# EvolEcolGroup/tidypopgen

Hardware: AMD Instinct MI355X
Metric: SNP-genotypes/s (N x M) for IBS+KING+GRM+Fst+PCA; max |delta| vs CPU ref (cpu_baseline.parity) (higher is better)
Workload: dtype fp4-e2m1 operands (exact integers, f32 accumulate) for the cross-products, the PCA Gram and the grouped counts, int8 (int32 accumulate) for the loadings, f64 for statistics

## Files before the change

tidypopgen_amd/csrc/pca.hip:

```cpp
#include <math.h>
#include <stdio.h>
#include <stdlib.h>
#include <string.h>
#include <time.h>

#include <algorithm>

#include "common.h"
#include <type_traits>
#include "devfrag.h"

#define MFMA_I8(a, b, c) __builtin_amdgcn_mfma_i32_32x32x32_i8((a), (b), (c), 0, 0, 0)
#define PCA_NAN __longlong_as_double(0x7FF8000000000000ll)

__global__ void tpg_pca_center_scale_kernel(const int4* __restrict__ counts, int64_t m, int64_t n,
                                            double* __restrict__ center, double* __restrict__ scale,
                                            int* __restrict__ flags) {
  for (int64_t j = blockIdx.x * (int64_t)blockDim.x + threadIdx.x; j < m; j += (int64_t)gridDim.x * blockDim.x) {
    const int4 c = counts[j];
    if (c.w != 0) flags[0] = 1;
    const double mean = (double)(c.y + 2 * c.z) / (double)n;
    const double p = mean / 2;
    const double sd = sqrt(2 * p * (1 - p));
    if (!(sd > 0)) flags[1] = 1;
// ... 963 lines not shown
      for (int c = 0; c < 8; c++) {
        const int j = cg * 8 + c;
        const double x = j < p ? xs[i + j * p] : 0.0;
        a0[c] += a * x;
        a1[c] += y * x;
      }
    }
#pragma unroll
  for (int c = 0; c < 8; c++) {
    const int j = cg * 8 + c;
    double r = 0;
    if (live && j < p) {
      Y0[row + (int64_t)j * n] = a0[c];
      Y1[row + (int64_t)j * n] = a1[c];
      r = ldexp(a1[c] - theta[j] * a0[c], -e1);
      r *= r;
    }
#pragma unroll
    for (int off = 16; off >= 1; off >>= 1) r += __shfl_xor(r, off, 32);
    if ((threadIdx.x & 31) == 0 && j < p) rpart[(int64_t)blockIdx.x * p + j] = r;
  }
}

__global__ void tpg_fill_random_kernel(double* __restrict__ Q, int64_t total, uint64_t seed) {
  for (int64_t idx = blockIdx.x * (int64_t)blockDim.x + threadIdx.x; idx < total; idx += (int64_t)gridDim.x * blockDim.x) {
    uint64_t x = (uint64_t)idx * 0x9E3779B97F4A7C15ull + seed;
    x = (x ^ (x >> 30)) * 0xBF58476D1CE4E5B9ull;
    x = (x ^ (x >> 27)) * 0x94D049BB133111EBull;
    x ^= x >> 31;
    Q[idx] = (double)(int64_t)(x >> 11) * (1.0 / 9007199254740992.0) - 0.5;
  }
}

#include "host/host_eig.h"

struct EigWork {
  tpg_ctx* ctx;
  const double* K;
  int n, b, S;
  double *part = nullptr, *gpart = nullptr;
  int nchunks, rows_per_chunk;
  const double* L = nullptr;
  int nl = 0;
  double *lam_dev = nullptr, *cdev = nullptr, *dtmp = nullptr;
  double* xdev = nullptr;
  DevArena mem;
  TpgPcaOp* op = nullptr;
  int init() {
    const int row_blocks = (n + 63) / 64;
    S = 1;
    while (row_blocks * S < 4 * ctx->num_cu && S < 32 && n / (S * 2) >= 64) S *= 2;
    S = std::max(1, std::min((int)S, 2 * ctx->num_cu / row_blocks));
    if (op) S = 1;
    rows_per_chunk = n <= 4096 ? 32 : 64;
    nchunks = (n + rows_per_chunk - 1) / rows_per_chunk;
    TPG_TRY(mem.get(&part, (size_t)S * (size_t)b * (size_t)n));
    TPG_TRY(mem.get(&gpart, (size_t)nchunks * 64 * 64));
    TPG_TRY(mem.get(&lam_dev, 64));
    TPG_TRY(mem.get(&cdev, 64 * 64));
    TPG_TRY(mem.get(&dtmp, (size_t)b * (size_t)n));
    TPG_TRY(mem.get(&xdev, 64 * 64 + 64));
    return TPG_OK;
  }
  int set_locked(const double* Lptr, int count, const double* lam_host) {
    L = Lptr;
    nl = count;
    if (count > 0) TPG_HIP(tpg_push_small(ctx, lam_dev, lam_host, sizeof(double) * (size_t)count));
    return TPG_OK;
  }
  int apply(const double* Q, double alpha, const double* Y1, double beta, const double* Y0, double gamma, double* Y) {
    if (op) {
      TPG_TRY(tpg_pcaop_apply(ctx, op, Q, b, part));
    } else {
      dim3 grid((unsigned)((n + 63) / 64), (unsigned)S);
      TPG_LAUNCH(ctx, "eig_symm_apply", tpg_symm_apply_kernel, grid, dim3(256), 0, K, n, Q, b, S, part);
    }
    const double* Dm = nullptr;
    if (nl > 0) {
      TPG_LAUNCH(ctx, "eig_gram_small", tpg_gram_small_kernel, dim3((unsigned)nchunks), dim3(256), 0, L, nl, Q, b, n,
                 rows_per_chunk, gpart);
      TPG_LAUNCH(ctx, "eig_gram_reduce", tpg_gram_reduce_kernel, dim3((unsigned)((nl * b + 63) / 64)), dim3(256), 0,
                 (const double*)gpart, nchunks, nl, b, (const double*)lam_dev, cdev);
      TPG_LAUNCH(ctx, "eig_right_mult", tpg_right_mult_kernel, dim3((unsigned)((n + 31) / 32)), dim3(256), 0, L, n, nl,
                 (const double*)cdev, b, dtmp);
      Dm = dtmp;
    }
    TPG_LAUNCH(ctx, "eig_combine", tpg_combine_kernel, dim3(1024), dim3(256), 0, (const double*)part, S,
               (int64_t)n * b, alpha, Y1, beta, Y0, gamma, Y, Dm);
    TPG_CHECK_LAUNCH();
    return TPG_OK;
  }
  int gram(const double* A, int p, const double* B, int bb, std::vector<double>& C) {
    TPG_LAUNCH(ctx, "eig_gram_small", tpg_gram_small_kernel, dim3((unsigned)nchunks), dim3(256), 0, A, p, B, bb, n,
               rows_per_chunk, gpart);
    TPG_LAUNCH(ctx, "eig_gram_reduce", tpg_gram_reduce_kernel, dim3((unsigned)((p * bb + 63) / 64)), dim3(256), 0,
               (const double*)gpart, nchunks, p, bb, (const double*)nullptr, cdev);
    C.assign((size_t)p * bb, 0.0);
    TPG_HIP(tpg_fetch_small(ctx, C.data(), cdev, sizeof(double) * (size_t)p * bb));
    return TPG_OK;
  }
  int ritz(const double* A, const double* Yk, int p, const std::vector<double>& X, const std::vector<double>& theta, int e1,
           double* Y0, double* Y1, std::vector<double>& res2) {
    double* dx = xdev;
    TPG_HIP(tpg_push_small(ctx, dx, X.data(), sizeof(double) * (size_t)p * p));
    TPG_HIP(tpg_push_small(ctx, dx + 64 * 64, theta.data(), sizeof(double) * (size_t)p));
    const int nblk = (n + 31) / 32;
    TPG_LAUNCH(ctx, "eig_ritz", tpg_ritz_kernel, dim3((unsigned)nblk), dim3(256), 0, A, Yk, n, p, (const double*)dx,
               (const double*)(dx + 64 * 64), e1, Y0, Y1, gpart);
    TPG_LAUNCH(ctx, "eig_gram_reduce", tpg_gram_reduce_kernel, dim3((unsigned)((p + 63) / 64)), dim3(256), 0,
               (const double*)gpart, nblk, p, 1, (const double*)nullptr, cdev);
    res2.assign((size_t)p, 0.0);
    TPG_HIP(tpg_fetch_small(ctx, res2.data(), cdev, sizeof(double) * (size_t)p));
    return TPG_OK;
  }
  int rmult(const double* A, int p, const std::vector<double>& X, int b2, double* Y) {
    double* dx = xdev;
    TPG_HIP(tpg_push_small(ctx, dx, X.data(), sizeof(double) * (size_t)p * b2));
    TPG_LAUNCH(ctx, "eig_right_mult", tpg_right_mult_kernel, dim3((unsigned)((n + 31) / 32)), dim3(256), 0, A, n, p,
               (const double*)dx, b2, Y);
    TPG_CHECK_LAUNCH();
    return TPG_OK;
  }
};

struct StageTimer {
  tpg_ctx* ctx; const char* tag; bool on; double t0;
  static double now() { struct timespec ts; clock_gettime(CLOCK_MONOTONIC, &ts); return ts.tv_sec * 1e3 + ts.tv_nsec * 1e-6; }
  StageTimer(tpg_ctx* c, const char* t) : ctx(c), tag(t), on(tpg_env_set("TPG_DEBUG")), t0(0) { if (on) { (void)hipStreamSynchronize(ctx->stream); t0 = now(); } }
  void mark(const char* what) {
    if (!on) return;
    (void)hipStreamSynchronize(ctx->stream);
    const double t1 = now();
    fprintf(stderr, "[%s] %-28s %8.3f ms\n", tag, what, t1 - t0);
    t0 = t1;
  }
};

static int eig_topk(tpg_ctx* ctx, const double* d_K, int n, int k, double* lambda_host, double* d_U, double tol = 1e-12,
                    const double* d_P = nullptr, int np_ = 0, double* lam1_io = nullptr, TpgPcaOp* op = nullptr) {
  int b = 2 * k + 12;
  b = tpg_env_int("TPG_EIG_BLOCK", b);
  if (b > 64) b = 64;
  if (b > n - np_) b = n - np_;
  TPG_REQUIRE(k <= b, TPG_EINVAL, "k = %d too large (at most %d components)", k, b);
  TPG_REQUIRE(!op || b <= op->bmax, TPG_EINVAL, "block of %d columns, operator scratch for %d", b, op->bmax);
  EigWork w{ctx, d_K, n, b, 1};
  w.op = op;
  TPG_TRY(w.init());
  double *Q = nullptr, *Y = nullptr, *Y0 = nullptr, *Y1 = nullptr;
  for (double** blk : {&Q, &Y, &Y0, &Y1}) TPG_TRY(w.mem.get(blk, (size_t)n * (size_t)b));
  auto colbytes = [&](int cols) { return sizeof(double) * (size_t)n * (size_t)cols; };
  auto axpby = [&](const double* x, double alpha, const double* y, double beta, double* out, int cols) -> int {
    TPG_LAUNCH(ctx, "eig_combine", tpg_combine_kernel, dim3(1024), dim3(256), 0, x, 1, (int64_t)n * cols, alpha, y,
               beta, (const double*)nullptr, 0.0, out, (const double*)nullptr);
    TPG_CHECK_LAUNCH();
    return TPG_OK;
  };

  auto project_earlier = [&](double* A, int cols, double* tmp) -> int {
    for (int c0 = 0; c0 < np_; c0 += 64) {
      const int pc = std::min(64, np_ - c0);
      const double* P = d_P + (size_t)n * (size_t)c0;
      std::vector<double> Cm;
      TPG_TRY(w.gram(P, pc, A, cols, Cm));
      TPG_TRY(w.rmult(P, pc, Cm, cols, tmp));
      TPG_TRY(axpby(tmp, -1.0, A, 1.0, A, cols));
    }
    return TPG_OK;
  };

  auto orthonormalize = [&](double* A, int act, const double* L, int nl, double* tmp, int passes = 2) -> int {
    int extra_passes = 0;
    for (int pass = 0; pass < passes; pass++) {
      TPG_TRY(project_earlier(A, act, tmp));
      if (nl > 0) {
        std::vector<double> Cm;
        TPG_TRY(w.gram(L, nl, A, act, Cm));
        TPG_TRY(w.rmult(L, nl, Cm, act, tmp));
        TPG_TRY(axpby(tmp, -1.0, A, 1.0, A, act));
      }
      std::vector<double> G, Ri;
      TPG_TRY(w.gram(A, act, A, act, G));
      std::vector<double> D((size_t)act);
      for (int j = 0; j < act; j++) D[(size_t)j] = G[j + (size_t)j * act] > 0 ? 1.0 / sqrt(G[j + (size_t)j * act]) : 1.0;
      for (int j = 0; j < act; j++)
        for (int i = 0; i < act; i++) G[i + (size_t)j * act] *= D[(size_t)i] * D[(size_t)j];
      std::vector<double> Gsave = G;
      if (host_cholesky_upper(G, act)) {
        host_upper_inverse(G, act, Ri);
      } else {
        std::vector<double> lamg, Vg;
        host_sym_eig(Gsave, act, lamg, Vg);
        if (tpg_env_set("TPG_DEBUG")) fprintf(stderr, "[eig] CholQR fell back to the eigen-decomposition of the block Gram matrix\n");
        const double floor_ = std::max(lamg[0], 1e-300) * 1e-14;
        Ri.assign((size_t)act * act, 0.0);
        for (int j = 0; j < act; j++) {
          const double sc = 1.0 / sqrt(std::max(lamg[(size_t)j], floor_));
          for (int i = 0; i < act; i++) Ri[i + (size_t)j * act] = Vg[i + (size_t)j * act] * sc;
        }
        if (pass == passes - 1) pass = passes - 2, extra_passes++;
        if (extra_passes > 3) { tpg_set_error("eigen solver: block lost rank"); return TPG_ENUMERIC; }
      }
      for (int j = 0; j < act; j++)
        for (int i = 0; i < act; i++) Ri[i + (size_t)j * act] *= D[(size_t)i];
      TPG_TRY(w.rmult(A, act, Ri, act, tmp));
      TPG_HIP(tpg_copy_dev(ctx, A, tmp, colbytes(act)));
    }
    return TPG_OK;
  };

  StageTimer st(ctx, "eig");
  TPG_LAUNCH(ctx, "eig_random", tpg_fill_random_kernel, dim3(512), dim3(256), 0, Q, (int64_t)n * b, (uint64_t)0x5EED);
  TPG_TRY(orthonormalize(Q, b, nullptr, 0, Y, np_ > 0 ? 2 : 1));
  st.mark("init + orthonormalize");
  std::vector<double> lam((size_t)b, 0.0), theta, X, H;
  int nl = 0;
  const int MAXIT = 200;
  const double TOL = tol, AMP = 1e6;
  const bool own_scale = !(lam1_io && *lam1_io > 0);
  double lam1 = own_scale ? 0 : *lam1_io;
  int e1 = 0;
  for (int it = 0; it < MAXIT && nl < k; it++) {
    const int act = b - nl;
    double* A = Q + (size_t)n * nl;
    w.b = act;
    TPG_TRY(w.set_locked(Q, nl, lam.data()));
    TPG_TRY(w.apply(A, 1.0, nullptr, 0, nullptr, 0, Y));
    TPG_TRY(project_earlier(Y, act, Y0));
    TPG_TRY(w.gram(A, act, Y, act, H));
    st.mark("apply + gram(H)");
    for (int i = 0; i < act; i++)
      for (int j = i + 1; j < act; j++) {
        const double sy = 0.5 * (H[i + (size_t)j * act] + H[j + (size_t)i * act]);
        H[i + (size_t)j * act] = sy;
        H[j + (size_t)i * act] = sy;
      }
    const bool first = it == 0 && b < n - np_;
    host_sym_eig(H, act, theta, X, !first);
    st.mark("host_sym_eig");
    std::vector<double> RR;
    if (first) {
      if (own_scale) lam1 = fabs(theta[0]) > 0 ? fabs(theta[0]) : 1.0;
    } else {
      if (own_scale && nl == 0) lam1 = fabs(theta[0]) > 0 ? fabs(theta[0]) : 1.0;
      frexp(lam1, &e1);
      TPG_TRY(w.ritz(A, Y, act, X, theta, e1, Y0, Y1, RR));
      TPG_HIP(tpg_copy_dev(ctx, A, Y0, colbytes(act)));
      st.mark("ritz vectors + residuals");
    }
    const double lam1s = ldexp(lam1, -e1);
    int newly = 0;
    while (!first && newly < act && nl + newly < k && sqrt(std::max(0.0, RR[(size_t)newly])) < TOL * lam1s) newly++;
    for (int j = 0; j < newly; j++) lam[(size_t)(nl + j)] = theta[(size_t)j];
    nl += newly;
    if (nl >= k) break;
    const int act2 = b - nl;
    TPG_REQUIRE(act2 >= 2, TPG_ENUMERIC, "eigen solver ran out of active vectors");
    double* A2 = Q + (size_t)n * nl;
    const double* KA2 = first ? Y : Y1 + (size_t)n * newly;
    const double up = std::max(theta[(size_t)act - 1], 1e-300 * lam1), lo = 0.0;
    const double a0 = std::max(theta[(size_t)newly], up * (1 + 1e-8));
    const double ec = (up - lo) / 2, cc = (up + lo) / 2;
    const double x0 = (a0 - cc) / ec;
    int deg = 20;
    if (x0 > 1.0 + 1e-12) {
      const double dmax = log(2 * AMP) / acosh(x0);
      deg = dmax < 2 ? 2 : (dmax > 20 ? 20 : (int)dmax);
    }
    if (tpg_env_set("TPG_DEBUG"))
      fprintf(stderr, "[eig] it %d act %d locked %d (+%d) deg %d theta_first %.4g theta_last %.4g lam1 %.4g res0 %.3g\n", it,
              act, nl, newly, deg, theta[(size_t)newly], theta[(size_t)act - 1], lam1,
              first ? -1.0 : sqrt(std::max(0.0, RR[(size_t)newly])) / lam1s);
    w.b = act2;
    TPG_TRY(w.set_locked(Q, nl, lam.data()));
    double sigma = ec / (a0 - cc);
    const double sigma1 = sigma;
    double* prev = Y0;
    double* cur = first ? Y1 : Y;
    double* nxt = first ? Y : Y1;
    TPG_HIP(tpg_copy_dev(ctx, prev, A2, colbytes(act2)));
    TPG_LAUNCH(ctx, "eig_combine", tpg_combine_kernel, dim3(1024), dim3(256), 0, KA2, 1, (int64_t)n * act2,
               sigma1 / ec, (const double*)prev, -cc * sigma1 / ec, (const double*)nullptr, 0.0, cur,
               (const double*)nullptr);
    for (int dgr = 2; dgr <= deg; dgr++) {
      const double sigma2 = 1.0 / (2.0 / sigma1 - sigma);
      TPG_TRY(w.apply(cur, 2 * sigma2 / ec, cur, -2 * sigma2 * cc / ec, prev, -sigma * sigma2, nxt));
      double* t = prev; prev = cur; cur = nxt; nxt = t;
      sigma = sigma2;
    }
    TPG_HIP(tpg_copy_dev(ctx, A2, cur, colbytes(act2)));
    st.mark("chebyshev filter");
    TPG_TRY(orthonormalize(A2, act2, Q, nl, prev));
    st.mark("orthonormalize");
  }
  TPG_REQUIRE(nl >= k, TPG_ENUMERIC, "eigen solver did not converge (%d of %d pairs)", nl, k);
  for (int j = 0; j < k; j++) lambda_host[j] = lam[(size_t)j];
  if (lam1_io) *lam1_io = lam1;
  TPG_HIP(tpg_copy_dev(ctx, d_U, Q, colbytes(k)));
  return TPG_OK;
}

static int pca_loadings_device(tpg_ctx* ctx, const tpg_view* v, const double* d_center, const double* d_scale,
                               const double* d_U, const double* d_dk, int k, double* d_V);

__global__ __launch_bounds__(256) void tpg_deflate_kernel(double* __restrict__ K, int n, const double* __restrict__ U,
                                                          const double* __restrict__ lam, int kb) {
  __shared__ double ui[16][33], uj[16][33];
  const int tx = threadIdx.x & 15, ty = threadIdx.x >> 4;
  const int i0 = blockIdx.x * 16, j0 = blockIdx.y * 16;
  for (int q = threadIdx.x; q < 16 * kb; q += 256) {
    const int r = q & 15, c = q >> 4;
    ui[r][c] = i0 + r < n ? U[(int64_t)(i0 + r) + (int64_t)c * n] * lam[c] : 0.0;
    uj[r][c] = j0 + r < n ? U[(int64_t)(j0 + r) + (int64_t)c * n] : 0.0;
  }
  __syncthreads();
  const int i = i0 + tx, j = j0 + ty;
  if (i >= n || j >= n) return;
  double s = 0.0;
  for (int c = 0; c < kb; c++) s = fma(ui[tx][c], uj[ty][c], s);
  K[(int64_t)i + (int64_t)j * n] -= s;
}

static int eig_topk_any(tpg_ctx* ctx, const double* d_K, int n, int k, double* lambda_host, double* d_U, double tol) {
  if (k <= 52) return eig_topk(ctx, d_K, n, k, lambda_host, d_U, tol);
  DevBuf b_Kw, b_lam;
  TPG_TRY(b_Kw.alloc_n<double>((size_t)n * (size_t)n));
  TPG_TRY(b_lam.alloc_n<double>(32));
  double *const Kw = b_Kw.as<double>(), *const d_lam = b_lam.as<double>();
  TPG_HIP(hipMemcpyAsync(Kw, d_K, sizeof(double) * (size_t)n * (size_t)n, hipMemcpyDeviceToDevice, ctx->stream));
  const int KB = 26;
  double lam1 = 0;
  for (int done = 0; done < k;) {
    const int kb = std::min(KB, k - done);
    double* Ub = d_U + (size_t)done * (size_t)n;
    TPG_TRY(eig_topk(ctx, Kw, n, kb, lambda_host + done, Ub, tol, d_U, done, &lam1));
    done += kb;
    if (done < k) {
      TPG_HIP(tpg_h2d_async(ctx, d_lam, lambda_host + done - kb, sizeof(double) * (size_t)kb));
      TPG_LAUNCH(ctx, "eig_deflate", tpg_deflate_kernel, dim3((unsigned)((n + 15) / 16), (unsigned)((n + 15) / 16)), dim3(256), 0, Kw, n,
                 (const double*)Ub, (const double*)d_lam, kb);
      TPG_CHECK_LAUNCH();
    }
  }
  return TPG_OK;
}

static int pca_svd_impl(tpg_ctx* ctx, tpg_comm* comm, const tpg_view* v, int k, double tol, double* d, double* u,
                        double* vload, double* center, double* scale, double* square_frobenius);

extern "C" int tpg_pca_partial_svd(tpg_ctx* ctx, const tpg_view* v, int k, double* d, double* u, double* vload,
                                   double* center, double* scale, double* square_frobenius) {
  TpgEnter _enter(ctx);
  return pca_svd_impl(ctx, nullptr, v, k, 1e-12, d, u, vload, center, scale, square_frobenius);
}

extern "C" int tpg_pca_partial_svd_sharded(tpg_ctx* ctx, tpg_comm* comm, const tpg_view* v, int k, double* d, double* u,
                                           double* vload, double* center, double* scale, double* square_frobenius) {
  TpgEnter _enter(ctx);
  TPG_REQUIRE(comm && comm->ctx == ctx, TPG_EINVAL, "bad communicator");
  return pca_svd_impl(ctx, comm, v, k, 1e-12, d, u, vload, center, scale, square_frobenius);
}

extern "C" int tpg_pca_random_svd(tpg_ctx* ctx, const tpg_view* v, int k, double tol, double* d, double* u,
                                  double* vload, double* center, double* scale, double* square_frobenius) {
  TpgEnter _enter(ctx);
  TPG_REQUIRE(tol > 0 && tol < 1, TPG_EINVAL, "tol = %g out of (0, 1)", tol);
  return pca_svd_impl(ctx, nullptr, v, k, tol < 1e-12 ? 1e-12 : tol, d, u, vload, center, scale, square_frobenius);
}

static int pca_op_block(int64_t n, int k, bool env) {
  int b = 2 * k + 12;
  if (env) b = tpg_env_int("TPG_EIG_BLOCK", b);
  if (b > 64) b = 64;
  if (b > n) b = (int)n;
  return b < 1 ? 1 : b;
}

extern "C" size_t tpg_pca_op_scratch_bytes(int64_t n, int64_t m, int k) {
  if (n < 1 || m < 1 || k < 1 || k > 52) return 0;
  const size_t b = (size_t)pca_op_block(n, k, false), nn = (size_t)n, mm = (size_t)m, kk = (size_t)k;
  const size_t rows_per_chunk = n <= 4096 ? 32 : 64, nchunks = (nn + rows_per_chunk - 1) / rows_per_chunk;
  size_t total = tpg_pcaop_work_bytes(n, m, (int)b, 256);
  total += sizeof(double) * (6 * nn * b + nchunks * 64 * 64 + 3 * 64 * 64 + 128);
  total += sizeof(int32_t) * 4 * mm + sizeof(double) * (2 * mm + nn * kk + mm * kk + kk);
  const size_t CT = (kk * 6  + 31) / 32;
  total += (size_t)ceil_div(n, 128) * 4 * CT * 1024 + (size_t)ceil_div(m, 128) * 128 * CT * 32 * sizeof(int32_t);
  return total;
}

extern "C" int tpg_pca_gram_route_fits(tpg_ctx* ctx, int64_t n, int k, int* fits) {
  TpgEnter _enter(ctx);
  TPG_REQUIRE(ctx && fits, TPG_EINVAL, "null argument");
  TPG_REQUIRE(n >= 1 && k >= 1, TPG_EINVAL, "bad n = %lld / k = %d", (long long)n, k);
  size_t fr = 0, tot = 0;
  TPG_HIP(hipMemGetInfo(&fr, &tot));
  const double need = 8.0 * (double)n * (double)n + 8.0 * 37.0 * (double)n * (double)pca_op_block(n, std::min(k, 26), false);
  *fits = need <= 0.5 * (double)fr ? 1 : 0;
  return TPG_OK;
}

extern "C" int tpg_pca_random_svd_op(tpg_ctx* ctx, const tpg_view* v, int k, double tol, double* d, double* u, double* vload,
                                     double* center, double* scale, double* square_frobenius, int* n_apply) {
  TpgEnter _enter(ctx);
  TPG_REQUIRE(ctx && v && d && u && vload && center && scale, TPG_EINVAL, "null argument");
  TPG_REQUIRE(tol >= TPG_PCA_OP_TOL_FLOOR && tol < 1, TPG_EINVAL,
              "tol = %g out of [%g, 1): the operator products are exact to about 1e-11, a tighter tolerance takes the Gram route "
              "(tpg_pca_random_svd)", tol, (double)TPG_PCA_OP_TOL_FLOOR);
  TPG_REQUIRE(k >= 1 && k <= v->n && k <= v->m, TPG_EINVAL, "k = %d out of range", k);
  TPG_REQUIRE(k <= 52, TPG_EINVAL, "k = %d: the operator route takes at most 52 components, more take the Gram route "
              "(tpg_pca_random_svd)", k);
  TPG_REQUIRE(v->n <= 2147483647ll, TPG_EINVAL, "n = %lld too large", (long long)v->n);
  const int64_t n = v->n, m = v->m;
  OutBuf oc, os, ou, ov;
  TPG_TRY(oc.init(center, sizeof(double) * (size_t)m));
  TPG_TRY(os.init(scale, sizeof(double) * (size_t)m));
  TPG_TRY(ou.init(u, sizeof(double) * (size_t)n * (size_t)k));
  TPG_TRY(ov.init(vload, sizeof(double) * (size_t)m * (size_t)k));
  DevBuf b_counts, b_dk;
  TPG_TRY(b_counts.alloc_n<int32_t>(4 * (size_t)m));
  TPG_TRY(b_dk.alloc_n<double>((size_t)k));
  StageTimer st(ctx, "svd_op");
  TPG_TRY(pca_counts_center_scale(ctx, v, b_counts.as<int32_t>(), oc.dev<double>(), os.dev<double>()));
  if (square_frobenius)
    TPG_TRY(frobenius_from_counts(ctx, v, b_counts.as<int32_t>(), oc.dev<double>(), os.dev<double>(), square_frobenius));
  b_counts.free();
  st.mark("counts, center, scale, frobenius");
  std::vector<double> lam((size_t)k), dh((size_t)k);
  {
    TpgPcaOp op;
    TPG_TRY(tpg_pcaop_init(ctx, &op, v, oc.dev<double>(), os.dev<double>(), pca_op_block(n, k, true)));
    TPG_TRY(eig_topk(ctx, nullptr, (int)n, k, lam.data(), ou.dev<double>(), tol, nullptr, 0, nullptr, &op));
    if (n_apply) *n_apply = op.n_apply;
  }
  st.mark("eig_topk (operator)");
  for (int j = 0; j < k; j++) dh[(size_t)j] = sqrt(lam[(size_t)j] > 0 ? lam[(size_t)j] : 0.0);
  TPG_HIP(tpg_push_small(ctx, b_dk.as<double>(), dh.data(), sizeof(double) * (size_t)k));
  TPG_TRY(pca_loadings_device(ctx, v, oc.dev<double>(), os.dev<double>(), ou.dev<double>(), b_dk.as<double>(), k, ov.dev<double>()));
  if (tpg_is_device_ptr(d)) TPG_HIP(tpg_push_small(ctx, d, dh.data(), sizeof(double) * (size_t)k));
  else memcpy(d, dh.data(), sizeof(double) * (size_t)k);
  TPG_HIP(hipStreamSynchronize(ctx->stream));
  st.mark("loadings");
  TPG_TRY(oc.commit(ctx));
  TPG_TRY(os.commit(ctx));
  TPG_TRY(ou.commit(ctx));
  return ov.commit(ctx);
}

__global__ void tpg_tri_pack_kernel(const double* __restrict__ K, int n, double* __restrict__ tri) {
  const int64_t total = (int64_t)n * n;
  for (int64_t idx = blockIdx.x * (int64_t)blockDim.x + threadIdx.x; idx < total; idx += (int64_t)gridDim.x * blockDim.x) {
    const int64_t i = idx % n, k = idx / n;
    if (i <= k) tri[k * (k + 1) / 2 + i] = K[idx];
  }
}
__global__ void tpg_tri_unpack_kernel(const double* __restrict__ tri, int n, double* __restrict__ K) {
  const int64_t total = (int64_t)n * n;
  for (int64_t idx = blockIdx.x * (int64_t)blockDim.x + threadIdx.x; idx < total; idx += (int64_t)gridDim.x * blockDim.x) {
    const int64_t i = idx % n, k = idx / n;
    const int64_t lo = i < k ? i : k, hi = i < k ? k : i;
    K[idx] = tri[hi * (hi + 1) / 2 + lo];
  }
}

int tpg_pca_gram_allreduce(tpg_ctx* ctx, tpg_comm* comm, double* d_K, int64_t n) {
  if (!comm || !(comm->nranks > 1 || comm->nccl)) return TPG_OK;
  const int64_t ntri = n * (n + 1) / 2;
  DevBuf b_tri;
  int lrc = b_tri.alloc_n<double>((size_t)ntri);
  if (lrc != TPG_OK) (void)hipGetLastError();
  TPG_TRY(tpg_comm_agree(comm, lrc));
  double* const d_tri = b_tri.as<double>();
  TPG_LAUNCH(ctx, "pca_gram_tri", tpg_tri_pack_kernel, dim3(2048), dim3(256), 0, (const double*)d_K, (int)n, d_tri);
  {
    ProfScope ps(ctx, "pca_gram_allreduce");
    TPG_TRY(tpg_comm_allreduce(comm, d_tri, ntri, 1));
  }
  TPG_LAUNCH(ctx, "pca_gram_tri", tpg_tri_unpack_kernel, dim3(2048), dim3(256), 0, (const double*)d_tri, (int)n, d_K);
  return TPG_OK;
}

static int pca_svd_impl(tpg_ctx* ctx, tpg_comm* comm, const tpg_view* v, int k, double tol, double* d, double* u,
                        double* vload, double* center, double* scale, double* square_frobenius) {
  TPG_REQUIRE(ctx && v && d && u && vload && center && scale, TPG_EINVAL, "null argument");
  TPG_REQUIRE(k >= 1 && k <= v->n, TPG_EINVAL, "k = %d out of range", k);
  const int64_t n = v->n, m = v->m;
  OutBuf oc, os, ou, ov;
  int32_t* d_counts = nullptr;
  double *d_K = nullptr, *d_dk = nullptr, *d_tri = nullptr;
  DevBuf b_counts, b_K, b_dk, b_tri;
  StageTimer st(ctx, "svd");
  const bool exchange = comm && (comm->nranks > 1 || comm->nccl);
  const int64_t ntri = n * (n + 1) / 2;
  auto local_steps = [&]() -> int {
    TPG_REQUIRE(k <= m, TPG_EINVAL, "k = %d but this view has %lld loci", k, (long long)m);
    TPG_TRY(oc.init(center, sizeof(double) * (size_t)m));
    TPG_TRY(os.init(scale, sizeof(double) * (size_t)m));
    TPG_TRY(ou.init(u, sizeof(double) * (size_t)n * (size_t)k));
    TPG_TRY(ov.init(vload, sizeof(double) * (size_t)m * (size_t)k));
    TPG_TRY(b_counts.alloc_n<int32_t>(4 * (size_t)m));
    TPG_TRY(b_K.alloc_n<double>((size_t)n * (size_t)n));
    TPG_TRY(b_dk.alloc_n<double>((size_t)k));
    if (exchange) TPG_TRY(b_tri.alloc_n<double>((size_t)ntri));
    d_counts = b_counts.as<int32_t>();
    d_K = b_K.as<double>();
    d_dk = b_dk.as<double>();
    d_tri = b_tri.as<double>();
    TPG_TRY(pca_counts_center_scale(ctx, v, d_counts, oc.dev<double>(), os.dev<double>()));
    st.mark("counts, center, scale");
    if (square_frobenius) TPG_TRY(frobenius_from_counts(ctx, v, d_counts, oc.dev<double>(), os.dev<double>(), square_frobenius));
    return TPG_OK;
  };
  int lrc = local_steps();
  if (exchange) lrc = tpg_comm_agree(comm, lrc);
  TPG_TRY(lrc);
  if (square_frobenius && exchange) TPG_TRY(tpg_comm_allreduce_f64(ctx, comm, square_frobenius, 1));
  st.mark("frobenius + alloc K");
  auto gram_branch = [&]() -> int {
    bool exchanged = false;
    if (exchange) TPG_TRY(tpg_gram_classes_exchanged(ctx, comm, v, d_counts, os.dev<double>(), d_K, &exchanged));
    if (exchanged) return pca_double_center_inplace(ctx, d_K, n);
    return pca_gram_device(ctx, v, oc.dev<double>(), os.dev<double>(), d_K, true);
  };
  int grc = gram_branch();
  if (exchange) grc = tpg_comm_agree(comm, grc);
  TPG_TRY(grc);
  st.mark("gram");
  if (exchange) {
    TPG_LAUNCH(ctx, "pca_gram_tri", tpg_tri_pack_kernel, dim3(2048), dim3(256), 0, (const double*)d_K, (int)n, d_tri);
    {
      ProfScope ps(ctx, "pca_gram_allreduce");
      TPG_TRY(tpg_comm_allreduce(comm, d_tri, ntri, 1));
    }
    TPG_LAUNCH(ctx, "pca_gram_tri", tpg_tri_unpack_kernel, dim3(2048), dim3(256), 0, (const double*)d_tri, (int)n, d_K);
  }
  std::vector<double> lam((size_t)k);
  TPG_TRY(eig_topk_any(ctx, d_K, (int)n, k, lam.data(), ou.dev<double>(), tol));
  st.mark("eig_topk");
  std::vector<double> dh((size_t)k);
  for (int j = 0; j < k; j++) dh[(size_t)j] = sqrt(lam[(size_t)j] > 0 ? lam[(size_t)j] : 0.0);
  TPG_HIP(tpg_push_small(ctx, d_dk, dh.data(), sizeof(double) * (size_t)k));
  TPG_TRY(pca_loadings_device(ctx, v, oc.dev<double>(), os.dev<double>(), ou.dev<double>(), d_dk, k, ov.dev<double>()));
  if (tpg_is_device_ptr(d)) TPG_HIP(tpg_push_small(ctx, d, dh.data(), sizeof(double) * (size_t)k));
  else memcpy(d, dh.data(), sizeof(double) * (size_t)k);
  TPG_HIP(hipStreamSynchronize(ctx->stream));
  st.mark("loadings");
  TPG_TRY(oc.commit(ctx));
  TPG_TRY(os.commit(ctx));
  TPG_TRY(ou.commit(ctx));
  return ov.commit(ctx);
}

#define LD_TU 6

__global__ void tpg_u_digits_kernel(const double* __restrict__ U, int64_t n, int k, int FU, int64_t Q, int CT,
                                    uint4* __restrict__ UD) {
  const int64_t total = Q * 4 * CT * 64;
  for (int64_t idx = blockIdx.x * (int64_t)blockDim.x + threadIdx.x; idx < total;
       idx += (int64_t)gridDim.x * blockDim.x) {
    const int lane = (int)(idx & 63);
    const int64_t tq = idx >> 6;
    const int ct = (int)(tq % CT);
    const int64_t qs = tq / CT;
    const int s = (int)(qs & 3);
    const int64_t q = qs >> 2;
    const int col = 32 * ct + (lane & 31), h = lane >> 5;
    const int kk = col / LD_TU, t = col % LD_TU;
    uint32_t w[4] = {0, 0, 0, 0};
    if (kk < k)
      for (int e = 0; e < 16; e++) {
        const int64_t i = 128 * q + 32 * s + 16 * h + e;
        if (i >= n) continue;
        long long W = llrint(ldexp(U[i + (int64_t)kk * n], FU));
        long long dig = 0;
        for (int tt = 0; tt <= t; tt++) {
          dig = W & 127;
          if (dig >= 64) dig -= 128;
          W = (W - dig) >> 7;
        }
        w[e >> 2] |= (uint32_t)((int)dig & 0xFF) << (8 * (e & 3));
      }
    UD[idx] = make_uint4(w[0], w[1], w[2], w[3]);
  }
}

__global__ __launch_bounds__(256) void tpg_uq_colsum_kernel(const double* __restrict__ U, int64_t n, int FU,
                                                            double* __restrict__ usum) {
  __shared__ double sh[256];
  const int kk = blockIdx.x;
  double acc = 0;
  for (int64_t i = threadIdx.x; i < n; i += 256) acc += ldexp((double)llrint(ldexp(U[i + (int64_t)kk * n], FU)), -FU);
  sh[threadIdx.x] = acc;
  __syncthreads();
  for (int w = 128; w > 0; w >>= 1) {
    if ((int)threadIdx.x < w) sh[threadIdx.x] += sh[threadIdx.x + w];
    __syncthreads();
  }
  if (threadIdx.x == 0) usum[kk] = sh[0];
}

#ifndef LD_NLT
#define LD_NLT 2
#endif
#ifndef LD_WGS
#define LD_WGS 2
#endif
__device__ __forceinline__ int64_t tpg_uniform64_pca(int64_t x) {
  const uint32_t lo = __builtin_amdgcn_readfirstlane((uint32_t)x), hi = __builtin_amdgcn_readfirstlane((uint32_t)((uint64_t)x >> 32));
  return (int64_t)(((uint64_t)hi << 32) | lo);
}

template <int C, class F>
__device__ __forceinline__ void tpg_pca_static_for(F&& f) {
  if constexpr (C > 0) {
    tpg_pca_static_for<C - 1>(f);
    f(std::integral_constant<int, C - 1>{});
  }
}

template <int CTP, bool LMV>
__global__ __launch_bounds__(256, LD_WGS) void tpg_loadings_mfma_kernel(const uint4* __restrict__ L,
                                                                   const uint4* __restrict__ UD, int64_t n_lt,
                                                                   int64_t Q, int ct0, int CT,
                                                                   int32_t* __restrict__ out, int Cpad) {
  __shared__ __attribute__((aligned(16))) uint4 ubuf[2][4 * CTP][64];
  const int lane = threadIdx.x & 63, wv = threadIdx.x >> 6;
  const int64_t lt0 = ((int64_t)blockIdx.x * 4 + wv) * LD_NLT;
  v16i acc[LD_NLT][CTP];
#pragma unroll
  for (int t = 0; t < LD_NLT; t++)
#pragma unroll
    for (int c = 0; c < CTP; c++)
#pragma unroll
      for (int r = 0; r < 16; r++) acc[t][c][r] = 0;
  const int Qi = (int)Q;
  const int64_t lt0u = tpg_uniform64_pca(lt0);
  const char* pa[LD_NLT];
#pragma unroll
  for (int t = 0; t < LD_NLT; t++) pa[t] = (const char*)(L + ((lt0u + t < n_lt ? lt0u + t : 0) * Q) * 64);
  auto LDG = [&](const char* p, int blk) {
    uint32_t off = (uint32_t)lane * 16u + (uint32_t)blk * 1024u;
    asm("" : "+v"(off));
    return *(const uint4*)(p + off);
  };
  const int ldq = (lane >> 1) & 1;
  const uint32_t aoff = LMV ? (uint32_t)tpg_lm_piece(lane >> 2, Qi, 0, lane & 1) * 16u : (uint32_t)lane * 16u;
  auto LDA = [&](const char* p, int q, int X) {
    uint32_t off;
    if constexpr (LMV) off = aoff + (uint32_t)tpg_lm_piece(16 * X, Qi, q + ldq < Qi ? q + ldq : Qi - 1, 0) * 16u;
    else off = aoff + (uint32_t)q * 1024u;
    asm("" : "+v"(off));
    return *(const uint4*)(p + off);
  };
  const int lm_src = (((lane & 15) * 4 + ((lane >> 4) & 1) * 2 + (lane >> 5)) * 4);
  constexpr int LD_D = 4;
  static_assert(LD_D % 2 == 0, "the slot of a group's digit fragments is its parity");
  uint4 AR[LD_D][LD_NLT];
#pragma unroll
  for (int d = 0; d < (LMV ? 2 : LD_D - 1); d++)
#pragma unroll
    for (int t = 0; t < LD_NLT; t++) AR[d][t] = LMV ? LDA(pa[t], 0, d) : LDA(pa[t], d < Qi ? d : Qi - 1, 0);
  const char* pu = (const char*)(UD + ct0 * 64);
  uint4 un[2][CTP];
  auto ufrag = [&](int q, int j) {
    const int it = wv + 4 * j;
    return LDG(pu, (q * 4 + it / CTP) * CT + it % CTP);
  };
#pragma unroll
  for (int j = 0; j < CTP; j++) {
    ubuf[0][wv + 4 * j][lane] = ufrag(0, j);
    un[1][j] = ufrag(Qi > 1 ? 1 : 0, j);
  }
  tpg_lds_barrier();
  auto group = [&](auto Cc, auto Mm, int q) {
    constexpr int C = decltype(Cc)::value, M = decltype(Mm)::value;
    const int qa = q + LD_D - 1 < Qi ? q + LD_D - 1 : Qi - 1, qu = q + 2 < Qi ? q + 2 : Qi - 1;
    const int cur = q & 1;
    if constexpr (!LMV) {
#pragma unroll
      for (int t = 0; t < LD_NLT; t++) AR[M][t] = LDA(pa[t], qa, 0);
    } else if constexpr (C % 2 == 0) {
      static_assert(LD_D == 4, "a pair in use, a pair in flight");
      const int qb = q + 2 < Qi ? q + 2 : Qi - 1;
#pragma unroll
      for (int t = 0; t < LD_NLT; t++) {
        AR[(C + 2) % LD_D][t] = LDA(pa[t], qb, 0);
        AR[M][t] = LDA(pa[t], qb, 1);
      }
    }
    uint4 av[LD_NLT];
#pragma unroll
    for (int t = 0; t < LD_NLT; t++) {
      if constexpr (LMV) {
        constexpr int P = C & ~1, dq = C & 1;
        auto turn = [&](uint32_t a, uint32_t b) {
          const uint32_t bs = (uint32_t)__builtin_amdgcn_update_dpp(0, (int)b, 0x4E , 0xF, 0xF, true);
          return (uint32_t)__builtin_amdgcn_ds_bpermute(lm_src ^ (dq ? 8 : 0), (int)(ldq == dq ? a : bs));
        };
        av[t] = make_uint4(turn(AR[P][t].x, AR[P + 1][t].x), turn(AR[P][t].y, AR[P + 1][t].y), turn(AR[P][t].z, AR[P + 1][t].z),
                           turn(AR[P][t].w, AR[P + 1][t].w));
      } else {
        av[t] = AR[C][t];
      }
    }
#pragma unroll
    for (int j = 0; j < CTP; j++) un[C & 1][j] = ufrag(qu, j);
#pragma unroll
    for (int s = 0; s < 4; s++) {
      v4i fg[LD_NLT];
#pragma unroll
      for (int t = 0; t < LD_NLT; t++) {
        const uint32_t w = s == 0 ? av[t].x : s == 1 ? av[t].y : s == 2 ? av[t].z : av[t].w;
#pragma unroll
        for (int k = 0; k < 4; k++) fg[t][k] = (int)tpg_codes(w, k);
      }
#pragma unroll
      for (int c = 0; c < CTP; c++) {
        const uint4 bq = ubuf[cur][s * CTP + c][lane];
        v4i fb = {(int)bq.x, (int)bq.y, (int)bq.z, (int)bq.w};
#pragma unroll
        for (int t = 0; t < LD_NLT; t++) acc[t][c] = MFMA_I8(fg[t], fb, acc[t][c]);
      }
    }
#pragma unroll
    for (int j = 0; j < CTP; j++) ubuf[cur ^ 1][wv + 4 * j][lane] = un[(C & 1) ^ 1][j];
    tpg_lds_barrier();
  };
  for (int q = 0; q < Qi; q += LD_D)
    tpg_pca_static_for<LD_D>([&](auto kk) {
      constexpr int k = decltype(kk)::value;
      if (q + k < Qi) group(std::integral_constant<int, k>{}, std::integral_constant<int, (k + LD_D - 1) % LD_D>{}, q + k);
    });
#pragma unroll
  for (int t = 0; t < LD_NLT; t++) {
    if (lt0 + t >= n_lt) break;
#pragma unroll
    for (int c = 0; c < CTP; c++)
#pragma unroll
      for (int r = 0; r < 16; r++) {
        const int64_t row = (lt0 + t) * 32 + tpg_cd_row(r, lane);
        out[row * Cpad + 32 * (ct0 + c) + (lane & 31)] = acc[t][c][r];
      }
  }
}

__global__ void tpg_loadings_finalize_kernel(const int32_t* __restrict__ acc, int Cpad, int64_t m, int k, int FU,
                                             const double* __restrict__ center, const double* __restrict__ scale,
                                             const double* __restrict__ usum, const double* __restrict__ d,
                                             double* __restrict__ vload) {
  const int64_t total = m * k;
  for (int64_t idx = blockIdx.x * (int64_t)blockDim.x + threadIdx.x; idx < total;
       idx += (int64_t)gridDim.x * blockDim.x) {
    const int kk = (int)(idx % k);
    const int64_t j = idx / k;
    long long S = 0;
#pragma unroll
    for (int t = LD_TU - 1; t >= 0; t--) S = S * 128 + (long long)acc[j * Cpad + kk * LD_TU + t];
    const double gu = ldexp((double)S, -FU);
    vload[j + (int64_t)kk * m] = (gu - center[j] * usum[kk]) / (scale[j] * d[kk]);
  }
}

__global__ __launch_bounds__(1024) void tpg_absmax_kernel(const double* __restrict__ x, int64_t total, double* __restrict__ out) {
  __shared__ double sh[1024];
  double mx = 0;
  bool bad = false;
  for (int64_t i = threadIdx.x; i < total; i += 1024) {
    const double a = fabs(x[i]);
    if (a != a) bad = true;
    mx = a > mx ? a : mx;
  }
  sh[threadIdx.x] = bad ? __longlong_as_double(0x7FF8000000000000ll) : mx;
  __syncthreads();
  for (int w = 512; w > 0; w >>= 1) {
    if ((int)threadIdx.x < w) {
      const double a = sh[threadIdx.x], b = sh[threadIdx.x + w];
      sh[threadIdx.x] = (a != a || b != b) ? __longlong_as_double(0x7FF8000000000000ll) : (a > b ? a : b);
    }
    __syncthreads();
  }
  if (threadIdx.x == 0) out[0] = sh[0];
}

static int pca_loadings_device(tpg_ctx* ctx, const tpg_view* v, const double* d_center, const double* d_scale,
                               const double* d_U, const double* d_dk, int k, double* d_V) {
  const int64_t n = v->n, m = v->m;
  double amax = 0;
  {
    DevBuf d_amax;
    TPG_TRY(d_amax.alloc_n<double>(1));
    TPG_LAUNCH(ctx, "loadings_u_digits", tpg_absmax_kernel, dim3(1), dim3(1024), 0, d_U, n * (int64_t)k, d_amax.as<double>());
    TPG_HIP(tpg_fetch_small(ctx, &amax, d_amax.p, sizeof(double)));
  }
  TPG_REQUIRE(amax > 0 && amax == amax && amax < 1e300, TPG_ENUMERIC, "degenerate eigenvectors");
  int ex = 0;
  frexp(amax, &ex);
  const int FU = 7 * LD_TU - 2 - ex;
  const int CT = (int)ceil_div((int64_t)k * LD_TU, 32);
  const int Cpad = CT * 32;
  const int64_t n_lt = v->KG * 4;
  DevBuf b_UD, b_acc, b_usum;
  TPG_TRY(b_UD.alloc((size_t)v->Q * 4 * CT * 1024));
  TPG_TRY(b_acc.alloc_n<int32_t>((size_t)n_lt * 32 * (size_t)Cpad));
  TPG_TRY(b_usum.alloc_n<double>((size_t)k));
  uint4* const d_UD = b_UD.as<uint4>();
  int32_t* const d_acc = b_acc.as<int32_t>();
  double* const d_usum = b_usum.as<double>();
  TPG_LAUNCH(ctx, "loadings_u_digits", tpg_u_digits_kernel, dim3(1024), dim3(256), 0, d_U, n, k, FU, v->Q, CT, d_UD);
  TPG_LAUNCH(ctx, "loadings_u_digits", tpg_uq_colsum_kernel, dim3((unsigned)k), dim3(256), 0, d_U, n, FU, d_usum);
  const unsigned grid = (unsigned)ceil_div(n_lt, 4 * LD_NLT);
  if (!v->LM) TPG_TRY(tpg_view_need_L(ctx, v));
  for (int ct0 = 0; ct0 < CT;) {
    const int left = CT - ct0;
#define LD_LAUNCH(C)                                                                                             \
  do {                                                                                                           \
    if (v->LM)                                                                                                   \
      TPG_LAUNCH(ctx, "loadings_mfma", (tpg_loadings_mfma_kernel<C, true>), dim3(grid), dim3(256), 0,            \
                 (const uint4*)v->LM, (const uint4*)d_UD, n_lt, v->Q, ct0, CT, d_acc, Cpad);                     \
    else                                                                                                         \
      TPG_LAUNCH(ctx, "loadings_mfma", (tpg_loadings_mfma_kernel<C, false>), dim3(grid), dim3(256), 0,           \
                 (const uint4*)v->L, (const uint4*)d_UD, n_lt, v->Q, ct0, CT, d_acc, Cpad);                      \
  } while (0)
    if (left >= 4) { LD_LAUNCH(4); ct0 += 4; }
    else if (left == 3) { LD_LAUNCH(3); ct0 += 3; }
    else if (left == 2) { LD_LAUNCH(2); ct0 += 2; }
    else { LD_LAUNCH(1); ct0 += 1; }
#undef LD_LAUNCH
  }
  TPG_LAUNCH(ctx, "loadings_finalize", tpg_loadings_finalize_kernel, dim3(2048), dim3(256), 0, (const int32_t*)d_acc,
             Cpad, m, k, FU, d_center, d_scale, (const double*)d_usum, d_dk, d_V);
  TPG_CHECK_LAUNCH();
  TPG_HIP(hipStreamSynchronize(ctx->stream));
  return TPG_OK;
}

int tpg_sym_eig_topk_tol(tpg_ctx* ctx, const double* d_K, int64_t n, int k, double tol, double* lambda_host, double* d_U) {
  TPG_REQUIRE(ctx && d_K && lambda_host && d_U, TPG_EINVAL, "null argument");
  TPG_REQUIRE(n > 0 && k >= 1 && k <= n, TPG_EINVAL, "bad n = %lld / k = %d", (long long)n, k);
  return eig_topk_any(ctx, d_K, (int)n, k, lambda_host, d_U, tol);
}

extern "C" int tpg_sym_eig_topk(tpg_ctx* ctx, const double* K, int64_t n, int k, double* lambda, double* U) {
  TpgEnter _enter(ctx);
  TPG_REQUIRE(ctx && K && lambda && U, TPG_EINVAL, "null argument");
  TPG_REQUIRE(n > 0 && k >= 1 && k <= n, TPG_EINVAL, "bad n = %lld / k = %d", (long long)n, k);
  InBuf ik;
  TPG_TRY(ik.init(ctx, K, sizeof(double) * (size_t)n * (size_t)n));
  OutBuf ou;
  TPG_TRY(ou.init(U, sizeof(double) * (size_t)n * (size_t)k));
  std::vector<double> lam((size_t)k);
  TPG_TRY(eig_topk_any(ctx, ik.dev<double>(), (int)n, k, lam.data(), ou.dev<double>(), 1e-12));
  if (tpg_is_device_ptr(lambda)) TPG_HIP(hipMemcpyAsync(lambda, lam.data(), sizeof(double) * (size_t)k, hipMemcpyHostToDevice, ctx->stream));
  else memcpy(lambda, lam.data(), sizeof(double) * (size_t)k);
  TPG_HIP(hipStreamSynchronize(ctx->stream));
  return ou.commit(ctx);
}

extern "C" int tpg_pca_loadings(tpg_ctx* ctx, const tpg_view* v, const double* center, const double* scale,
                                const double* U, const double* d, int k, double* vload) {
  TpgEnter _enter(ctx);
  TPG_REQUIRE(ctx && v && center && scale && U && d && vload, TPG_EINVAL, "null argument");
  TPG_REQUIRE(k >= 1, TPG_EINVAL, "k must be positive");
  const int64_t n = v->n, m = v->m;
  InBuf ic, is, iu, id;
  TPG_TRY(ic.init(ctx, center, sizeof(double) * (size_t)m));
  TPG_TRY(is.init(ctx, scale, sizeof(double) * (size_t)m));
  TPG_TRY(iu.init(ctx, U, sizeof(double) * (size_t)n * (size_t)k));
  TPG_TRY(id.init(ctx, d, sizeof(double) * (size_t)k));
  OutBuf ov;
  TPG_TRY(ov.init(vload, sizeof(double) * (size_t)m * (size_t)k));
  DevBuf d_counts, d_flag;
  TPG_TRY(d_counts.alloc_n<int32_t>(4 * (size_t)m));
  TPG_TRY(d_flag.alloc_n<int>(2));
  int flag[2] = {0, 1};
  TPG_TRY(tpg_launch_loci_counts(ctx, v, d_counts.as<int32_t>()));
  TPG_HIP(hipMemsetAsync(d_flag.p, 0, 2 * sizeof(int), ctx->stream));
  TPG_LAUNCH(ctx, "pca_center_check", tpg_center_is_mean_kernel, dim3(1024), dim3(256), 0, (const int4*)d_counts.p,
             ic.dev<double>(), m, n, d_flag.as<int>());
  TPG_HIP(tpg_fetch_small(ctx, flag, d_flag.p, 2 * sizeof(int)));
  d_counts.free();
  d_flag.free();
  if (!flag[1]) {
    TPG_TRY(pca_loadings_device(ctx, v, ic.dev<double>(), is.dev<double>(), iu.dev<double>(), id.dev<double>(), k,
                                ov.dev<double>()));
  } else {
    DevBuf d_inv;
    TPG_TRY(d_inv.alloc_n<double>((size_t)m));
    TPG_LAUNCH(ctx, "inv_scale", tpg_inv_kernel, dim3(1024), dim3(256), 0, is.dev<double>(), m, d_inv.as<double>());
    TPG_TRY(tpg_view_need_L(ctx, v));
    TPG_TRY(run_sweep(ctx, SW_ROWSCALE, v->L, v->KG * 4, v->Q, m, n, ic.dev<double>(), d_inv.as<double>(), iu.dev<double>(), n, k,
                      ov.dev<double>(), id.dev<double>(), nullptr));
  }
  return ov.commit(ctx);
}
```

Before: 140.2 billion.

## Fuse loadings finalize into MFMA kernel epilogue and parallelize absmax

The int8 loadings MFMA kernel now reconstructs the base-128 digit sums and applies centering, scaling and division by singular values in its epilogue. It stages accumulators through swizzled shared memory, removing the global int32 accumulator buffer and the separate finalize kernel. Column tiles are regrouped per launch so that each launch holds whole components (up to 21), with digit generation done per launch. The absmax reduction is also split across up to 64 blocks plus a second pass. The costs are more shared memory and registers in the MFMA kernel and more launches for digit generation.

```diff
diff --git a/tidypopgen_amd/csrc/pca.hip b/tidypopgen_amd/csrc/pca.hip
--- a/tidypopgen_amd/csrc/pca.hip
+++ b/tidypopgen_amd/csrc/pca.hip
@@ -1289,6 +1289,7 @@
 
 static int pca_loadings_device(tpg_ctx* ctx, const tpg_view* v, const double* d_center, const double* d_scale,
                                const double* d_U, const double* d_dk, int k, double* d_V);
+static int ld_column_tiles(int k);
 
 __global__ __launch_bounds__(256) void tpg_deflate_kernel(double* __restrict__ K, int n, const double* __restrict__ U,
                                                           const double* __restrict__ lam, int kb) {
@@ -1370,8 +1371,7 @@
   size_t total = tpg_pcaop_work_bytes(n, m, (int)b, 256);
   total += sizeof(double) * (6 * nn * b + nchunks * 64 * 64 + 3 * 64 * 64 + 128);
   total += sizeof(int32_t) * 4 * mm + sizeof(double) * (2 * mm + nn * kk + mm * kk + kk);
-  const size_t CT = (kk * 6  + 31) / 32;
-  total += (size_t)ceil_div(n, 128) * 4 * CT * 1024 + (size_t)ceil_div(m, 128) * 128 * CT * 32 * sizeof(int32_t);
+  total += (size_t)ceil_div(n, 128) * 4 * (size_t)ld_column_tiles(k) * 1024;
   return total;
 }
 
@@ -1539,21 +1539,21 @@
 
 #define LD_TU 6
 
-__global__ void tpg_u_digits_kernel(const double* __restrict__ U, int64_t n, int k, int FU, int64_t Q, int CT,
-                                    uint4* __restrict__ UD) {
-  const int64_t total = Q * 4 * CT * 64;
+__global__ void tpg_u_digits_kernel(const double* __restrict__ U, int64_t n, int FU, int64_t Q, int CT, int ct0, int ctp,
+                                    int kk0, int nk, uint4* __restrict__ UD) {
+  const int64_t total = Q * 4 * ctp * 64;
   for (int64_t idx = blockIdx.x * (int64_t)blockDim.x + threadIdx.x; idx < total;
        idx += (int64_t)gridDim.x * blockDim.x) {
     const int lane = (int)(idx & 63);
     const int64_t tq = idx >> 6;
-    const int ct = (int)(tq % CT);
-    const int64_t qs = tq / CT;
+    const int ct = (int)(tq % ctp);
+    const int64_t qs = tq / ctp;
     const int s = (int)(qs & 3);
     const int64_t q = qs >> 2;
     const int col = 32 * ct + (lane & 31), h = lane >> 5;
-    const int kk = col / LD_TU, t = col % LD_TU;
+    const int kk = kk0 + col / LD_TU, t = col % LD_TU;
     uint32_t w[4] = {0, 0, 0, 0};
-    if (kk < k)
+    if (col < nk * LD_TU)
       for (int e = 0; e < 16; e++) {
         const int64_t i = 128 * q + 32 * s + 16 * h + e;
         if (i >= n) continue;
@@ -1566,7 +1566,7 @@
         }
         w[e >> 2] |= (uint32_t)((int)dig & 0xFF) << (8 * (e & 3));
       }
-    UD[idx] = make_uint4(w[0], w[1], w[2], w[3]);
+    UD[(qs * CT + ct0 + ct) * 64 + lane] = make_uint4(w[0], w[1], w[2], w[3]);
   }
 }
 
@@ -1607,9 +1607,14 @@
 template <int CTP, bool LMV>
 __global__ __launch_bounds__(256, LD_WGS) void tpg_loadings_mfma_kernel(const uint4* __restrict__ L,
                                                                    const uint4* __restrict__ UD, int64_t n_lt,
-                                                                   int64_t Q, int ct0, int CT,
-                                                                   int32_t* __restrict__ out, int Cpad) {
-  __shared__ __attribute__((aligned(16))) uint4 ubuf[2][4 * CTP][64];
+                                                                   int64_t Q, int ct0, int CT, int64_t m, int kk0, int nk, int FU,
+                                                                   const double* __restrict__ center,
+                                                                   const double* __restrict__ scale,
+                                                                   const double* __restrict__ usum,
+                                                                   const double* __restrict__ d, double* __restrict__ vload) {
+  __shared__ __attribute__((aligned(16))) uint4 smem[4 * CTP * 32 * 32 / 4];
+  static_assert(sizeof(smem) >= sizeof(uint4) * 2 * 4 * CTP * 64, "the fragment buffers fit");
+  uint4(*const ubuf)[4 * CTP][64] = reinterpret_cast<uint4(*)[4 * CTP][64]>(smem);
   const int lane = threadIdx.x & 63, wv = threadIdx.x >> 6;
   const int64_t lt0 = ((int64_t)blockIdx.x * 4 + wv) * LD_NLT;
   v16i acc[LD_NLT][CTP];
@@ -1717,33 +1722,56 @@
       constexpr int k = decltype(kk)::value;
       if (q + k < Qi) group(std::integral_constant<int, k>{}, std::integral_constant<int, (k + LD_D - 1) % LD_D>{}, q + k);
     });
+  int32_t* const ep = (int32_t*)smem + wv * (32 * CTP * 32);
+  const int jl = lane & 31, h = lane >> 5;
+  constexpr int LD_NKH = (32 * CTP / LD_TU + 1) / 2;
+  double us[LD_NKH], dk[LD_NKH];
+#pragma unroll
+  for (int i = 0; i < LD_NKH; i++) {
+    const int kk = kk0 + (2 * i + h < nk ? 2 * i + h : nk - 1);
+    us[i] = usum[kk];
+    dk[i] = d[kk];
+  }
+  double cj[LD_NLT], sj[LD_NLT];
+#pragma unroll
+  for (int t = 0; t < LD_NLT; t++) {
+    const int64_t j = (lt0 + t) * 32 + jl;
+    cj[t] = j < m ? center[j] : 0.0;
+    sj[t] = j < m ? scale[j] : 1.0;
+  }
 #pragma unroll
   for (int t = 0; t < LD_NLT; t++) {
     if (lt0 + t >= n_lt) break;
 #pragma unroll
     for (int c = 0; c < CTP; c++)
 #pragma unroll
-      for (int r = 0; r < 16; r++) {
-        const int64_t row = (lt0 + t) * 32 + tpg_cd_row(r, lane);
-        out[row * Cpad + 32 * (ct0 + c) + (lane & 31)] = acc[t][c][r];
+      for (int g = 0; g < 4; g++) {
+        const int col = 32 * c + jl;
+        const v4i w = {acc[t][c][4 * g], acc[t][c][4 * g + 1], acc[t][c][4 * g + 2], acc[t][c][4 * g + 3]};
+        *(v4i*)(ep + col * 32 + (((2 * g + h) ^ (col & 7)) * 4)) = w;
       }
-  }
-}
-
-__global__ void tpg_loadings_finalize_kernel(const int32_t* __restrict__ acc, int Cpad, int64_t m, int k, int FU,
-                                             const double* __restrict__ center, const double* __restrict__ scale,
-                                             const double* __restrict__ usum, const double* __restrict__ d,
-                                             double* __restrict__ vload) {
-  const int64_t total = m * k;
-  for (int64_t idx = blockIdx.x * (int64_t)blockDim.x + threadIdx.x; idx < total;
-       idx += (int64_t)gridDim.x * blockDim.x) {
-    const int kk = (int)(idx % k);
-    const int64_t j = idx / k;
-    long long S = 0;
-#pragma unroll
-    for (int t = LD_TU - 1; t >= 0; t--) S = S * 128 + (long long)acc[j * Cpad + kk * LD_TU + t];
-    const double gu = ldexp((double)S, -FU);
-    vload[j + (int64_t)kk * m] = (gu - center[j] * usum[kk]) / (scale[j] * d[kk]);
+    __builtin_amdgcn_fence(__ATOMIC_RELEASE, "workgroup");
+    __builtin_amdgcn_wave_barrier();
+    __builtin_amdgcn_fence(__ATOMIC_ACQUIRE, "workgroup");
+    const int64_t j = (lt0 + t) * 32 + jl;
+    if (j < m) {
+#pragma unroll
+      for (int i = 0; i < LD_NKH; i++) {
+        const int kl = 2 * i + h;
+        if (kl >= nk) break;
+        long long S = 0;
+#pragma unroll
+        for (int tt = LD_TU - 1; tt >= 0; tt--) {
+          const int col = kl * LD_TU + tt;
+          S = S * 128 + (long long)ep[col * 32 + ((((jl >> 2) ^ (col & 7)) * 4) + (jl & 3))];
+        }
+        const double gu = ldexp((double)S, -FU);
+        vload[j + (int64_t)(kk0 + kl) * m] = (gu - cj[t] * us[i]) / (sj[t] * dk[i]);
+      }
+    }
+    __builtin_amdgcn_fence(__ATOMIC_RELEASE, "workgroup");
+    __builtin_amdgcn_wave_barrier();
+    __builtin_amdgcn_fence(__ATOMIC_ACQUIRE, "workgroup");
   }
 }
 
@@ -1751,7 +1779,7 @@
   __shared__ double sh[1024];
   double mx = 0;
   bool bad = false;
-  for (int64_t i = threadIdx.x; i < total; i += 1024) {
+  for (int64_t i = blockIdx.x * (int64_t)1024 + threadIdx.x; i < total; i += (int64_t)gridDim.x * 1024) {
     const double a = fabs(x[i]);
     if (a != a) bad = true;
     mx = a > mx ? a : mx;
@@ -1765,7 +1793,19 @@
     }
     __syncthreads();
   }
-  if (threadIdx.x == 0) out[0] = sh[0];
+  if (threadIdx.x == 0) out[blockIdx.x] = sh[0];
+}
+
+static int ld_launch_components(int launch, int left) { return left <= 21 ? left : launch < 15 ? 21 : 16; }
+static int ld_tiles_of(int nk) { return (nk * LD_TU + 31) / 32; }
+static int ld_column_tiles(int k) {
+  int CT = 0;
+  for (int kk0 = 0, launch = 0; kk0 < k; launch++) {
+    const int nk = ld_launch_components(launch, k - kk0);
+    CT += ld_tiles_of(nk);
+    kk0 += nk;
+  }
+  return CT;
 }
 
 static int pca_loadings_device(tpg_ctx* ctx, const tpg_view* v, const double* d_center, const double* d_scale,
@@ -1773,48 +1813,54 @@
   const int64_t n = v->n, m = v->m;
   double amax = 0;
   {
+    const int64_t total = n * (int64_t)k;
+    const unsigned parts = (unsigned)std::min<int64_t>(64, ceil_div(total, (int64_t)1024));
     DevBuf d_amax;
-    TPG_TRY(d_amax.alloc_n<double>(1));
-    TPG_LAUNCH(ctx, "loadings_u_digits", tpg_absmax_kernel, dim3(1), dim3(1024), 0, d_U, n * (int64_t)k, d_amax.as<double>());
+    TPG_TRY(d_amax.alloc_n<double>(1 + (size_t)parts));
+    double* const d_part = d_amax.as<double>() + (parts > 1 ? 1 : 0);
+    TPG_LAUNCH(ctx, "loadings_u_digits", tpg_absmax_kernel, dim3(parts), dim3(1024), 0, d_U, total, d_part);
+    if (parts > 1)
+      TPG_LAUNCH(ctx, "loadings_u_digits", tpg_absmax_kernel, dim3(1), dim3(1024), 0, (const double*)d_part, (int64_t)parts,
+                 d_amax.as<double>());
     TPG_HIP(tpg_fetch_small(ctx, &amax, d_amax.p, sizeof(double)));
   }
   TPG_REQUIRE(amax > 0 && amax == amax && amax < 1e300, TPG_ENUMERIC, "degenerate eigenvectors");
   int ex = 0;
   frexp(amax, &ex);
   const int FU = 7 * LD_TU - 2 - ex;
-  const int CT = (int)ceil_div((int64_t)k * LD_TU, 32);
-  const int Cpad = CT * 32;
+  const int CT = ld_column_tiles(k);
   const int64_t n_lt = v->KG * 4;
-  DevBuf b_UD, b_acc, b_usum;
+  DevBuf b_UD, b_usum;
   TPG_TRY(b_UD.alloc((size_t)v->Q * 4 * CT * 1024));
-  TPG_TRY(b_acc.alloc_n<int32_t>((size_t)n_lt * 32 * (size_t)Cpad));
   TPG_TRY(b_usum.alloc_n<double>((size_t)k));
   uint4* const d_UD = b_UD.as<uint4>();
-  int32_t* const d_acc = b_acc.as<int32_t>();
   double* const d_usum = b_usum.as<double>();
-  TPG_LAUNCH(ctx, "loadings_u_digits", tpg_u_digits_kernel, dim3(1024), dim3(256), 0, d_U, n, k, FU, v->Q, CT, d_UD);
   TPG_LAUNCH(ctx, "loadings_u_digits", tpg_uq_colsum_kernel, dim3((unsigned)k), dim3(256), 0, d_U, n, FU, d_usum);
   const unsigned grid = (unsigned)ceil_div(n_lt, 4 * LD_NLT);
   if (!v->LM) TPG_TRY(tpg_view_need_L(ctx, v));
-  for (int ct0 = 0; ct0 < CT;) {
-    const int left = CT - ct0;
+  for (int kk0 = 0, ct0 = 0, launch = 0; kk0 < k; launch++) {
+    const int nk = ld_launch_components(launch, k - kk0), ctp = ld_tiles_of(nk);
+    TPG_LAUNCH(ctx, "loadings_u_digits", tpg_u_digits_kernel, dim3(1024), dim3(256), 0, d_U, n, FU, v->Q, CT, ct0, ctp, kk0, nk,
+               d_UD);
 #define LD_LAUNCH(C)                                                                                             \
   do {                                                                                                           \
     if (v->LM)                                                                                                   \
       TPG_LAUNCH(ctx, "loadings_mfma", (tpg_loadings_mfma_kernel<C, true>), dim3(grid), dim3(256), 0,            \
-                 (const uint4*)v->LM, (const uint4*)d_UD, n_lt, v->Q, ct0, CT, d_acc, Cpad);                     \
+                 (const uint4*)v->LM, (const uint4*)d_UD, n_lt, v->Q, ct0, CT, m, kk0, nk, FU, d_center, d_scale, \
+                 (const double*)d_usum, d_dk, d_V);                                                              \
     else                                                                                                         \
       TPG_LAUNCH(ctx, "loadings_mfma", (tpg_loadings_mfma_kernel<C, false>), dim3(grid), dim3(256), 0,           \
-                 (const uint4*)v->L, (const uint4*)d_UD, n_lt, v->Q, ct0, CT, d_acc, Cpad);                      \
+                 (const uint4*)v->L, (const uint4*)d_UD, n_lt, v->Q, ct0, CT, m, kk0, nk, FU, d_center, d_scale, \
+                 (const double*)d_usum, d_dk, d_V);                                                              \
   } while (0)
-    if (left >= 4) { LD_LAUNCH(4); ct0 += 4; }
-    else if (left == 3) { LD_LAUNCH(3); ct0 += 3; }
-    else if (left == 2) { LD_LAUNCH(2); ct0 += 2; }
-    else { LD_LAUNCH(1); ct0 += 1; }
+    if (ctp == 4) LD_LAUNCH(4);
+    else if (ctp == 3) LD_LAUNCH(3);
+    else if (ctp == 2) LD_LAUNCH(2);
+    else LD_LAUNCH(1);
 #undef LD_LAUNCH
-  }
-  TPG_LAUNCH(ctx, "loadings_finalize", tpg_loadings_finalize_kernel, dim3(2048), dim3(256), 0, (const int32_t*)d_acc,
-             Cpad, m, k, FU, d_center, d_scale, (const double*)d_usum, d_dk, d_V);
+    kk0 += nk;
+    ct0 += ctp;
+  }
   TPG_CHECK_LAUNCH();
   TPG_HIP(hipStreamSynchronize(ctx->stream));
   return TPG_OK;
```

Result: no change. 141.2 billion (median of 6 runs) (+0.8%).
